# SebastianAment/CompressedSensing.jl

Hardware: AMD Instinct MI355X
Metric: OMP atoms selected/sec at m=4096,n=65536,k=256 (single-signal sweeps, 2 x 3 signals pipelined) (higher is better)
Workload: dtype f64; 1 GPU; configs[1]: single-signal OMP, A 4096x65536 Float32 Gaussian unit-norm, k=256, planted +-1 256-sparse x0 + noise 5e-3, eps=eps(Float32); signals_per_gpu=78, signals_in_flight=6, collective=none (one rank)

## Files before the change

compressedsensing.jl_amd/_lib.py:

```python
import ctypes as C
import os

import numpy as np

HERE = os.path.dirname(os.path.abspath(__file__))
LIB_PATH = os.path.join(HERE, "csrc", "libcsmp.so")

OK, EINVAL, EDIM, ERANGE, EHIP, ESTATE, ENOMEM, ERCCL, EIO = 0, -1, -2, -3, -4, -5, -6, -7, -8
F32, F64 = 0, 1
HOST, DEVICE, HOST_STREAMED = 0, 1, 2
ALGO_MP, ALGO_OMP, ALGO_GOMP, ALGO_FR, ALGO_SP, ALGO_OMPR = 0, 1, 2, 3, 4, 5
STOP_EPS, STOP_STAG, STOP_FULL = 1, 2, 4
OPT_BATCH_CERT, OPT_BATCH_GRAM, OPT_BATCH_WINDOW, OPT_PIPELINE, OPT_SOLVES_IN_FLIGHT, OPT_SCREENED_SWEEP, OPT_BATCH_SCREEN = 1, 2, 3, 4, 9, 10, 11
OPTIONS = {"batch_cert": OPT_BATCH_CERT, "batch_gram": OPT_BATCH_GRAM, "batch_window": OPT_BATCH_WINDOW, "pipeline": OPT_PIPELINE,
           "solves_in_flight": OPT_SOLVES_IN_FLIGHT, "screened_sweep": OPT_SCREENED_SWEEP, "batch_screen": OPT_BATCH_SCREEN}

i64 = C.c_int64
vp = C.c_void_p

SIGNATURES = {
    "csmp_version": (C.c_int, []),
    "csmp_create": (C.c_int, [C.POINTER(vp), C.c_int]),
    "csmp_destroy": (C.c_int, [vp]),
    "csmp_last_error": (C.c_char_p, [vp]),
# ... 70 lines not shown
    "csmp_profile_enable": (C.c_int, [vp, C.c_int]),
    "csmp_profile_read": (C.c_int, [vp, C.POINTER(i64), C.POINTER(C.c_double), C.c_int]),
    "csmp_bench_sweep": (C.c_int, [vp, C.c_int, C.c_int, C.POINTER(C.c_double)]),
    "csmp_bench_ard_forms": (C.c_int, [vp, C.c_int, C.c_int, C.c_double, C.POINTER(C.c_double), C.POINTER(C.c_double)]),
    "csmp_bp_rowgram": (C.c_int, [vp, vp, C.c_int]),
    "csmp_profile_overhead": (C.c_int, [vp, C.c_int, C.POINTER(C.c_double)]),
    "csmp_live_resources": (C.c_int, [C.POINTER(i64)] * 6),
    "csmp_profile_window": (C.c_int, [vp, C.POINTER(i64), C.POINTER(C.c_double), C.POINTER(C.c_double), C.POINTER(C.c_int)]),
    "csmp_sweep_config": (C.c_int, [vp, C.POINTER(C.c_int), C.POINTER(C.c_int), C.POINTER(C.c_int), C.POINTER(C.c_int), C.POINTER(i64), C.POINTER(C.c_int), C.POINTER(C.c_int)]),
    "csmp_sweep_group": (C.c_int, [vp, C.POINTER(C.c_int)]),
    "csmp_sweep_group_wide": (C.c_int, [vp, C.POINTER(C.c_int)]),
    "csmp_tune": (C.c_int, [vp, C.c_int, i64]),
    "csmp_batch_layout": (C.c_int, [vp, C.POINTER(i64), C.POINTER(C.c_int)]),
    "csmp_batch_screen_kernel": (C.c_char_p, [vp]),
}
TUNE = {"sweep_grid": 2, "sweep_unit": 3, "tick_grid": 4, "batch_budget_mib": 5, "diag_split": 6, "swap_refuse": 7, "rebuild_direct": 8, "sweep_dyn": 9, "tick_order": 10, "claim_pools": 11, "pipelines": 12, "pair_lds_kib": 13, "pair_split": 14, "sweep_lds_kib": 15, "sweep_short": 16, "phase_rows": 17, "fail_alloc": 18, "screen_static": 19, "group_max": 20, "group_wide": 21, "rowgram_scalar": 22}

COMM_ID_BYTES = 128
BABEL_KMAX = 1024
ARD_KMAX = 1024
REWEIGHT_CANDES, REWEIGHT_ARD = 0, 1
BP_CONVERGED, BP_FACTORED = 1, 2
BPD_CONVERGED, BPD_FACTORED = 1, 2
BPD_RHO = 100.0


def live_resources():
    v = [i64(0) for _ in range(6)]
    rc = lib().csmp_live_resources(*[C.byref(x) for x in v])
    if rc != OK:
        raise CsmpError(rc, "csmp_live_resources")
# ... 777 lines not shown
```

compressedsensing.jl_amd/csrc/csmp_kernels.hpp:

```cpp
#pragma once
#include <hip/hip_runtime.h>
#include <type_traits>
#include <stdint.h>

namespace csmp {

constexpr int kWave = 64;
constexpr int kSweepThreads = 256;
constexpr int kCPW = 4;
constexpr int kSlabRows = 64;
constexpr int kQrThreads = 256;

enum : int { STOP_EPS = 1, STOP_STAG = 2, STOP_FULL = 4, STOP_REORTH = 8 };
constexpr int STOP_UNCERTAIN = 256;

struct DevState {
    int nsel;
    int j;
    int cand;
    int go;
    int done;
    int steps;
    int go2;
    int pcount;
// ... 1845 lines not shown
    for (int i = 0; i < R; ++i) acc[0][i] = acc[1][i] = 0.0;
    const int Ni = (int)N;
    double bestv[NS];
    int besti[NS];
    double cst[NS];
    int ccst[NS];
#pragma unroll
    for (int s = 0; s < NS; ++s) {
        bestv[s] = -1.0;
        besti[s] = 0x7fffffff;
        cst[s] = 0.0;
        ccst[s] = -1;
    }
    int cslot = 0;
    auto cv = [&](const int i) { return mo ? p.cvec[kGroupMax + i] : p.cvec[i]; };
    auto flush = [&](const int s) {
        double* dst;
        bool on;
        if (s < S4) {
            dst = (lane & 32) ? cv(2 * s + 1) : cv(2 * s);
            on = (live >> (2 * s + (lane >> 5))) & 1u;
        } else {
            dst = cv(R - 1);
            on = (live >> (R - 1)) & 1u;
        }
        if (on && ccst[s] >= 0) dst[ccst[s]] = cst[s];
        ccst[s] = -1;
    };
    int64_t iq = q0, cq = q0;
    int ib = 0, cb = 0;
// ... 137 lines not shown
            for (int s = 0; s < NS; ++s) {
                double v;
                int col;
                bool mine;
                if (s < S4) {
                    v = row_xsum(xs16(xs32(acc[0][2 * s], acc[0][2 * s + 1]), xs32(acc[1][2 * s], acc[1][2 * s + 1])));
                    col = c0 + ((lane >> 4) & 1);
                    mine = ((lane ^ cslot) & 15) == 0;
                } else {
                    v = xs32(acc[0][R - 1], acc[1][R - 1]);
                    v = row_xsum(xs16(v, v));
                    col = c0 + (lane >> 5);
                    mine = ((lane ^ cslot) & 31) == 0;
                }
                const bool have = col < Ni;
                if (mine) {
                    cst[s] = v;
                    ccst[s] = have ? col : -1;
                }
                const double av = fabs(v);
                if (have && av > bestv[s]) {
                    bestv[s] = av;
                    besti[s] = col;
                }
            }
#pragma unroll
            for (int i = 0; i < R; ++i) acc[0][i] = acc[1][i] = 0.0;
            ++cslot;
            if ((cslot & 15) == 0) {
#pragma unroll
                for (int s = 0; s < S4; ++s) flush(s);
                if (cslot == 32) {
                    if constexpr (NS > S4) flush(S4);
                    cslot = 0;
                }
            }
            cb = 0;
            cq += stride;
        }
        --cleft;
    };
    if (T >= 2 * NB) {
        const int64_t groups = T / NB - 1;
        for (int64_t g = 0; g < groups; ++g) {
#pragma unroll
            for (int d = 0; d < NB; ++d) step(buf[d], std::true_type{});
        }
    }
    while (cleft > 0) {
#pragma unroll
        for (int d = 0; d < NB; ++d) {
            if (cleft == 0) break;
            step(buf[d], std::false_type{});
            if (ileft > 0) issue(buf[d]);
        }
    }
#pragma unroll
    for (int s = 0; s < NS; ++s) flush(s);
#pragma unroll
    for (int s = 0; s < S4; ++s) {
        if ((lane & 15) == 0) {
            const int e = (2 * s + (lane >> 5)) * 4 * NW + wave * 4 + ((lane >> 4) & 1);
            redv[e] = redv[e + 2] = bestv[s];
            redi[e] = redi[e + 2] = besti[s];
        }
    }
    if constexpr (NS > S4)
        argmax_put_rows(redv + (R - 1) * 4 * NW, redi + (R - 1) * 4 * NW, wave, lane, bestv[S4], besti[S4]);
    __syncthreads();
    if (tid < R && (live & (1u << tid)))
        argmax_reduce(redv + tid * 4 * NW, redi + tid * 4 * NW, 4 * NW, p.pval[mo + tid], p.pidx[mo + tid], bid);
}
template <typename TA, int U, int R>
// ... 38 lines not shown
    const int64_t ncol = col0 < N ? (N - 1 - col0) / stride + 1 : 0;
    double bestv[R];
    int besti[R];
    const int nunit = (Mv + UR - 1) / UR;
    const int Mst = nunit * UR;
    VT buf[NB][U];
    double acc[R];
#pragma unroll
    for (int i = 0; i < R; ++i) {
        bestv[i] = -1.0;
        besti[i] = 0x7fffffff;
        acc[i] = 0.0;
    }
    CStage<R> cs;
    cs.init();
    int64_t icol = col0, ccol = col0;
    int ib = 0, cb = 0;
    const int64_t T = ncol * nunit;
    int64_t ileft = T, cleft = T;
    auto issue = [&](VT(&b)[U]) {
        load_unit<TA, U>(A, icol, ld, ib * (U * kWave), nvec, lane, b);
        if (++ib == nunit) {
            ib = 0;
            icol += stride;
        }
        --ileft;
    };
#pragma unroll
    for (int d = 0; d < NB; ++d) {
        if (ileft <= 0) {
// ... 40 lines not shown
            } else {
                const double a0 = (double)b[u].x, a1 = (double)b[u].y;
#pragma unroll
                for (int i = 0; i < R; ++i) {
                    const f64x2* rs = reinterpret_cast<const f64x2*>(lds + (size_t)i * KP);
                    const f64x2 r01 = rs[t * kWave + lane];
                    acc[i] = fma(a0, r01.x, acc[i]);
                    acc[i] = fma(a1, r01.y, acc[i]);
                }
            }
        }
        if (++cb == nunit) {
#pragma unroll
            for (int i = 0; i < R; ++i) {
                const double c = wave_xsum(acc[i]);
                cs.put(lane, i, c);
                const double av = fabs(c);
                if (av > bestv[i]) {
                    bestv[i] = av;
                    besti[i] = (int)ccol;
                }
                acc[i] = 0.0;
            }
            cs.col(lane, ccol);
            cs.next(1, p.cvec, live);
            cb = 0;
            ccol += stride;
        }
        --cleft;
    };
    if (T >= 2 * NB) {
        const int64_t groups = T / NB - 1;
        for (int64_t g = 0; g < groups; ++g) {
#pragma unroll
            for (int d = 0; d < NB; ++d) {
                consume(buf[d]);
                issue(buf[d]);
            }
        }
    }
    while (cleft > 0) {
#pragma unroll
        for (int d = 0; d < NB; ++d) {
            if (cleft == 0) break;
            consume(buf[d]);
            if (ileft > 0) issue(buf[d]);
        }
    }
    cs.flush(p.cvec, live);
#pragma unroll
    for (int i = 0; i < R; ++i) argmax_put_rows(redv + i * 4 * NW, redi + i * 4 * NW, wave, lane, bestv[i], besti[i]);
    __syncthreads();
    if (tid < R && (live & (1u << tid)))
        argmax_reduce(redv + tid * 4 * NW, redi + tid * 4 * NW, 4 * NW, p.pval[tid], p.pidx[tid], bid);
}
template <typename TA, int U, int R>
__global__ __launch_bounds__(kSweepThreads) void k_sweep_multi_w4(const MultiSweep<TA> p) {
    extern __shared__ __attribute__((aligned(16))) double lds[];
    sweep_body_multi_w4<TA, U, 32 / U, R>(p, (int)blockIdx.x, lds);
}

template <typename TA>
struct GroupAppend {
    TickQr2 q2[kWideMax];
// ... 469 lines not shown
```

compressedsensing.jl_amd/csrc/host/batch_plan.hpp:

```cpp
#pragma once
#include <cstdint>
#include <vector>

struct TickStages {
    int z, y, x;
    bool az, ay, ax;
    int64_t tz;
};
static TickStages tick_stages(int64_t n, int64_t k, const int size[3]) {
    TickStages t;
    t.z = (int)(n % 3);
    t.y = (int)((n + 2) % 3);
    t.x = (int)((n + 1) % 3);
    t.tz = (n - t.z) / 3;
    t.az = size[t.z] > 0 && t.tz < k;
    t.ay = size[t.y] > 0 && n >= 1 + t.y && (n - 1 - t.y) / 3 < k;
    t.ax = size[t.x] > 0 && n >= 2 + t.x && (n - 2 - t.x) / 3 < k;
    return t;
}

enum class BatchSchedule {
    Signals,
    One,
    Pairs,
// ... 9 lines not shown
    PlanGroup g[2][3];
};

static std::vector<PlanGroup> even_groups(int64_t nsig, int R) {
    std::vector<PlanGroup> groups;
    if (nsig < 1 || R < 1) return groups;
    const int64_t ngroups = (nsig + R - 1) / R, base = nsig / ngroups, extra = nsig % ngroups;
    int64_t at = 0;
    for (int64_t i = 0; i < ngroups; ++i) {
        groups.push_back({at, (int)(base + (i < extra ? 1 : 0))});
        at += groups.back().size;
    }
    return groups;
}

static std::vector<PlanRound> batch_plan(int64_t nsig, BatchSchedule sched, int R, bool one_pipe = false) {
    std::vector<PlanRound> rounds;
    auto round = [&](RoundForm form) -> PlanRound& {
        rounds.emplace_back();
        rounds.back().form = form;
        return rounds.back();
    };
    int64_t at = 0;
    switch (sched) {
        case BatchSchedule::Signals: break;
        case BatchSchedule::One:
            for (; at < nsig; at += 3) {
                PlanRound& r = round(RoundForm::One);
                for (int g = 0; g < 3 && at + g < nsig; ++g) r.g[0][g] = {at + g, 1};
            }
            break;
// ... 1 lines not shown
            for (; nsig - at >= 6; at += 6) {
                PlanRound& r = round(RoundForm::Pair);
                for (int g = 0; g < 3; ++g) {
                    r.g[0][g] = {at + g, 1};
                    r.g[1][g] = {at + 3 + g, 1};
                }
            }
            for (; nsig - at >= 2; at += 2) {
                PlanRound& r = round(RoundForm::Pair);
                r.g[0][0] = {at, 1};
                r.g[1][0] = {at + 1, 1};
            }
            if (at < nsig) round(RoundForm::One).g[0][0] = {at, 1};
            break;
        case BatchSchedule::Grouped: {
            const std::vector<PlanGroup> groups = even_groups(nsig, R);
            for (size_t i = 0; i < groups.size(); ++i) {
                const size_t per = one_pipe ? 3 : 6;
                if (i % per == 0) round(RoundForm::Grouped);
                if (one_pipe) rounds.back().g[0][i % 3] = groups[i];
                else rounds.back().g[i % 2][(i % 6) / 2] = groups[i];
            }
            break;
        }
    }
    return rounds;
}

struct MpRound {
    PlanGroup g[2];
};
// ... 17 lines not shown
```

compressedsensing.jl_amd/csrc/host/ctx.hpp:

```cpp
static std::string g_create_err;
static constexpr int kRsEqCap = 4096;
static constexpr int kRsSettle = 256;

struct Solver {
    std::vector<int> hpos;
    std::vector<unsigned> hstamp;
    unsigned hgen = 0;
    int kcap = 0, outcap = 0;
    int qcap = 0;
    int64_t ldq = 0;
    int G = 0, Mpad = 0;
    double *b = nullptr, *r = nullptr, *cvec = nullptr, *pval = nullptr;
    int* pidx = nullptr;
    double *Q = nullptr, *R = nullptr, *z = nullptr, *W1 = nullptr, *P1 = nullptr, *P2 = nullptr, *P2s = nullptr, *P1s = nullptr;
    double *avec = nullptr, *vvec = nullptr, *coef = nullptr, *scal = nullptr;
    int *sel = nullptr, *cands = nullptr, *ncands = nullptr;
    double *top_lv = nullptr, *cvals = nullptr;
    int *top_li = nullptr, *rs_gt = nullptr, *rs_eq = nullptr, *rs_work = nullptr;
    RsState* rs = nullptr;
    int top_nb = 0;
    DevState* st = nullptr;
    double* bstage = nullptr;
    int64_t *out_idx = nullptr, *out_order = nullptr, *out_nnz = nullptr;
    double* out_val = nullptr;
// ... 188 lines not shown
    bool sweep_dyn = false;
    int tune_sweep_dyn = 0;
    int tune_pair_lds_kib = 0;
    int tune_pair_split = 0;
    int tune_fail_alloc = 0;
    int tune_pipelines = 0;
    int tune_group_max = 0;
    int sweep_group = 0;
    int tune_group_wide = 0;
    bool wide_refused = false;
    int group_wide = 0;
    int claim_pools = 8;
    int tune_rebuild_direct = 0;
    int tune_swap_refuse = 0;
    int tune_rowgram_scalar = 0;
    int tune_diag_split = 0;
    int64_t tune_batch_budget_mib = 0;
    void* comm = nullptr;
    int comm_rank = 0, comm_world = 1;
    int opt_batch_cert = 1;
    int opt_batch_gram = 0;
    int opt_batch_window = 0;
    int64_t scr_solves = 0, scr_fallbacks = 0;
    int scr_grid = 0;
    double scr_cert_abs = 0.0, scr_cert_rel = 0.0, scr_cert_abs2 = 0.0;
    int scr_kwin = 0;
    int scr_image = 1;
    bool scr_lone = false;
    int opt_screened = 0;
    int opt_batch_screen = 3;
// ... 109 lines not shown
```

compressedsensing.jl_amd/csrc/host/forward.hpp:

```cpp
struct FrPass {
    int nq = 1;
    const double* q1 = nullptr;
    double s1 = -1.0;
    const double* q2 = nullptr;
    double s2 = 1.0;
    int64_t qstride = 0;
    const int* unmark = nullptr;
    int update_only = 0;
};

template <typename TA, int U, bool FULL, int NQ>
static hipError_t fr_sweep_launch_t(csmp_ctx* ctx, const FrPass& ps, int grid, size_t lds, double max_eps, int skipmask) {
    Solver& s = ctx->s;
    auto kern = k_fr_sweep<TA, U, FULL, NQ>;
    if (lds > 64 * 1024) {
        hipError_t e = hipFuncSetAttribute((const void*)kern, hipFuncAttributeMaxDynamicSharedMemorySize, (int)lds);
        if (e != hipSuccess) return e;
    }
    hipLaunchKernelGGL(kern, dim3(grid), dim3(kSweepThreads), lds, ctx->stream, (const TA*)ctx->dA, ctx->ld, ctx->Mv, ctx->N,
                       (const double*)s.r, (const double*)s.Q, s.ldq, ps.q1, ps.s1, ps.q2, ps.s2, ps.unmark, ps.update_only, s.rho2,
                       s.dvec, s.pval, s.pidx, (const int*)s.sel, s.st, max_eps, skipmask);
    return hipGetLastError();
}
template <typename TA, int U, bool FULL>
// ... 310 lines not shown
                        if (!group) continue;
                        const int64_t sgn = r.g[p][g].first + m;
                        a.m[a.n++] = io.member(sv, sgn, sigflags + sgn);
                    }
                if (!group) {
                    PlanRound own = r;
                    for (int g = 0; g < 3; ++g) own.g[1 - p][g].size = 0;
                    CHECK(each_member(own, finish));
                } else if (a.n > 0) {
                    CHECK(twin_rc(ctx, cs[p], launch_finish_group(cs[p], a)));
                }
            }
            return CSMP_OK;
        };
        const int members = wide ? ctx->group_wide : ctx->sweep_group;
        for (const PlanRound& r : batch_plan(nsig, sched, members, wide && ctx->tune_group_wide == 2)) {
            CHECK(each_member(r, init));
            CHECK(ctx->dtype == CSMP_F32 ? run_round<float>(r, ctx, tw, isfr, k, eps, p2) : run_round<double>(r, ctx, tw, isfr, k, eps, p2));
            CHECK(finish_round(r));
        }
        return CSMP_OK;
    };
    if (sched == BatchSchedule::Signals) {
        for (int64_t sgn = 0; sgn < nsig && rc == CSMP_OK; ++sgn) rc = solve_one(sgn, true);
    } else {
        rc = batch_pipelines(ctx, twin, nslots, nslots_wide, 1, ensure, run_plan);
    }
    if (rc == CSMP_OK) {
        std::vector<int> hf((size_t)nsig);
        HIPCHECK(hipMemcpyAsync(hf.data(), sigflags, (size_t)nsig * sizeof(int), hipMemcpyDeviceToHost, ctx->stream));
        HIPCHECK(hipStreamSynchronize(ctx->stream));
// ... 128 lines not shown
```

compressedsensing.jl_amd/csrc/host/measure.hpp:

```cpp
extern "C" int csmp_profile_enable(csmp_ctx* ctx, int on) {
    if (!ctx) return CSMP_EINVAL;
    ctx->prof = on != 0;
    ctx->prof_every = on > 1 ? on : 1;
    ctx->prof_count = 0;
    ctx->prof_first = ctx->prof_last = -1;
    if (ctx->prof) {
        HIPCHECK(hipSetDevice(ctx->dev));
        if (!ctx->prof_ref) HIPCHECK(hipEventCreate(&ctx->prof_ref));
        HIPCHECK(hipEventRecord(ctx->prof_ref, ctx->stream));
    }
    return CSMP_OK;
}

extern "C" int csmp_profile_window(csmp_ctx* ctx, int64_t* launches, double* window_ms, double* mean_launch_ms, int* streams) {
    if (!ctx) return CSMP_EINVAL;
    HIPCHECK(hipSetDevice(ctx->dev));
    HIPCHECK(sync_all(ctx));
    csmp_ctx* cc[2] = {ctx, ctx->twins[0]};
    int64_t n = 0, pairs = 0;
    double t0 = 0.0, t1 = 0.0, dur = 0.0;
    int ns = 0;
    for (csmp_ctx* c : cc) {
        if (!c || c->ev_used < 2 || c->prof_first < 0 || !ctx->prof_ref) continue;
        if (c != ctx) HIPCHECK(hipStreamSynchronize(c->stream));
// ... 73 lines not shown
    std::lock_guard<std::mutex> g(csmp_track::mu);
    int64_t db = 0, pb = 0;
    for (const auto& kv : csmp_track::dev) db += (int64_t)kv.second;
    for (const auto& kv : csmp_track::pinned) pb += (int64_t)kv.second;
    if (device_bytes) *device_bytes = db;
    if (device_blocks) *device_blocks = (int64_t)csmp_track::dev.size();
    if (pinned_bytes) *pinned_bytes = pb;
    if (registered_ranges) *registered_ranges = (int64_t)csmp_track::registered.load();
    if (events) *events = (int64_t)csmp_track::events.load();
    if (streams) *streams = (int64_t)csmp_track::streams.load();
    return CSMP_OK;
}

template <typename TA>
static int bench_shared_sweep(csmp_ctx* ctx, int variant, int reps, double* avg_ms) {
    const int R = ctx->sweep_group, wide = variant >= 2;
    if (R < 1) return fail(ctx, CSMP_ESTATE, "bench_sweep: no shared sweep for this dictionary");
    if (wide && ctx->dtype != CSMP_F32) return fail(ctx, CSMP_ESTATE, "bench_sweep: the wide pass serves Float32 dictionaries");
    const int members = wide ? 2 * R : R;
    std::vector<double> r((size_t)ctx->M);
    uint64_t sd = 0x9E3779B97F4A7C15ull;
    int rc = CSMP_OK;
    for (int m = 0; m < members && rc == CSMP_OK; ++m) {
        activate_slot(ctx, 3 * m);
        rc = solver_ensure(ctx, 1, 1, false);
        ctx->s.begun = false;
        for (auto& v : r) {
            sd = sd * 6364136223846793005ull + 1442695040888963407ull;
            v = ((double)(sd >> 11) / 9007199254740992.0) - 0.5;
        }
        if (rc == CSMP_OK) rc = upload_b(ctx, r.data(), CSMP_F64);
    }
    activate_slot(ctx, 0);
    CHECK(rc);
    MultiSweep<TA> p;
    p.A = (const TA*)ctx->dA; p.ld = ctx->ld; p.Mv = ctx->Mv; p.N = ctx->N;
    p.eps = 0.0; p.check_eps = 0; p.skipmask = 0; p.KP = ctx->sweep_KP;
    p.nblk = wide ? wide_nblk(ctx) : pipe_nblk(ctx, ctx->dtype == CSMP_F32 ? kGroupTickGrid : kPairTickGrid);
    multi_members<TA>(ctx, p, 0, members);
    const size_t lds = std::max(sweep_multi_lds_bytes(p.KP, p.n), (size_t)kPairLdsKiB * 1024);
    auto launch = [&]() -> hipError_t { return wide ? wide_launch<TA>(ctx, p, lds, variant == 2) : multi_launch<TA>(ctx, p, lds); };
    for (int i = 0; i < 3; ++i) HIPCHECK(launch());
    struct Events {
        hipEvent_t e[2] = {nullptr, nullptr};
        ~Events() { for (hipEvent_t x : e) if (x) (void)hipEventDestroy(x); }
    } ev;
    HIPCHECK(hipEventCreate(&ev.e[0]));
    HIPCHECK(hipEventCreate(&ev.e[1]));
    HIPCHECK(hipEventRecord(ev.e[0], ctx->stream));
    for (int i = 0; i < reps; ++i) HIPCHECK(launch());
    HIPCHECK(hipEventRecord(ev.e[1], ctx->stream));
    HIPCHECK(hipStreamSynchronize(ctx->stream));
    float ms0 = 0.f;
    HIPCHECK(hipEventElapsedTime(&ms0, ev.e[0], ev.e[1]));
    if (avg_ms) *avg_ms = (double)ms0 / reps;
    return CSMP_OK;
}

extern "C" int csmp_bench_sweep(csmp_ctx* ctx, int variant, int reps, double* avg_ms) {
    if (!ctx || reps < 1) return CSMP_EINVAL;
    if (!ctx->dA) return fail(ctx, CSMP_ESTATE, "no dictionary set (csmp_set_dictionary)");
    if (variant < 0 || variant > 3) return fail(ctx, CSMP_ESTATE, "bench_sweep: variant 0 (the product kernel), 1 (the shared pass), 2 (the wide pass) or 3 (the wide pass, default-policy loads)");
    HIPCHECK(hipSetDevice(ctx->dev));
    if (variant != 0) return ctx->dtype == CSMP_F32 ? bench_shared_sweep<float>(ctx, variant, reps, avg_ms) : bench_shared_sweep<double>(ctx, variant, reps, avg_ms);
    CHECK(solver_ensure(ctx, 1, 1, false));
    ctx->s.begun = false;
    std::vector<double> r((size_t)ctx->M);
    uint64_t sd = 0x9E3779B97F4A7C15ull;
    for (auto& v : r) {
        sd = sd * 6364136223846793005ull + 1442695040888963407ull;
        v = ((double)(sd >> 11) / 9007199254740992.0) - 0.5;
    }
    CHECK(upload_b(ctx, r.data(), CSMP_F64));
    const bool was = ctx->prof;
    ctx->prof = false;
    for (int i = 0; i < 3; ++i) CHECK(launch_sweep(ctx, ctx->s.r, 0.0, 0, 0));
    hipEvent_t e0, e1;
// ... 60 lines not shown
            if (value < 0 || value > 64) return fail(ctx, CSMP_EINVAL, "csmp_tune: sweep_dyn must be 0 (static), 1 (every column claimed) or 2..64 (the last 1 / n of a workgroup's columns claimed)");
            ctx->tune_sweep_dyn = (int)value;
            break;
        case CSMP_TUNE_CLAIM_POOLS:
            if (value < 1 || value > 4096) return fail(ctx, CSMP_EINVAL, "csmp_tune: claim pools must be 1..4096");
            ctx->claim_pools = (int)value;
            return CSMP_OK;
        case CSMP_TUNE_PAIR_LDS_KIB:
            if (value > 159) return fail(ctx, CSMP_EINVAL, "csmp_tune: at most 159 KiB of LDS");
            ctx->tune_pair_lds_kib = (int)value;
            return CSMP_OK;
        case CSMP_TUNE_SCREEN_STATIC: ctx->tune_screen_static = value == 1 ? 1 : 0; return CSMP_OK;
        case CSMP_TUNE_PAIR_SPLIT: ctx->tune_pair_split = value == 1 ? 1 : 0; return CSMP_OK;
        case CSMP_TUNE_FAIL_ALLOC: ctx->tune_fail_alloc = (int)value; return CSMP_OK;
        case CSMP_TUNE_ROWGRAM_SCALAR: ctx->tune_rowgram_scalar = value == 1 ? 1 : 0; return CSMP_OK;
        case CSMP_TUNE_GROUP_MAX:
            if (value > kGroupMax) return fail(ctx, CSMP_EINVAL, "csmp_tune: group_max must be 0 (what the LDS holds) or 1 .. 4");
            ctx->tune_group_max = (int)value;
            break;
        case CSMP_TUNE_GROUP_WIDE:
            if (value > 2) return fail(ctx, CSMP_EINVAL, "csmp_tune: group_wide must be 0 (wide groups where they apply), 1 (off) or 2 (wide groups, three to a round on ONE pipeline)");
            ctx->tune_group_wide = (int)value;
            break;
        case CSMP_TUNE_PIPELINES:
            if (value > 3) return fail(ctx, CSMP_EINVAL, "csmp_tune: pipelines must be 0 (automatic), 1, 2 or 3");
            ctx->tune_pipelines = (int)value;
            return CSMP_OK;
        case CSMP_TUNE_TICK_ORDER: ctx->tick_sweep_first = value != 0; return CSMP_OK;
        case CSMP_TUNE_REBUILD_DIRECT: ctx->tune_rebuild_direct = value ? 1 : 0; return CSMP_OK;
        case CSMP_TUNE_SWAP_REFUSE: ctx->tune_swap_refuse = value ? 1 : 0; return CSMP_OK;
// ... 12 lines not shown
```

compressedsensing.jl_amd/csrc/host/mp_batch.hpp:

```cpp
constexpr bool kMpSplitLone = false;
template <typename TA>
static int mp_group_step(csmp_ctx* ctx, int size, int nblk, int nblk_wide, size_t lds_sweep) {
    CHECK(shared_pass_launch<TA>(ctx, 0, size, 0.0, 0, 0, nblk, nblk_wide, lds_sweep));
    const bool wide = size > kGroupMax;
    MpGroup g;
    g.n = size;
    for (int m = 0; m < kWideMax; ++m) {
        const Solver& s = *slot_ptr(ctx, 3 * std::min(m, size - 1));
        g.r[m] = s.r; g.cvec[m] = s.cvec; g.pval[m] = s.pval; g.pidx[m] = s.pidx; g.st[m] = s.st; g.sel[m] = s.sel; g.z[m] = s.z;
        g.cap[m] = s.kcap;
        g.nblk[m] = wide ? nblk_wide / 2 : nblk;
    }
    const int wgs = ((int)ctx->M + 255) / 256;
    hipLaunchKernelGGL(k_mp_group<TA>, dim3((unsigned)(size * wgs)), dim3(256), 0, ctx->stream, (const TA*)ctx->dA, ctx->ld, (int)ctx->M, ctx->N, g, wgs);
    HIPCHECK(hipGetLastError());
    return CSMP_OK;
}

static int mp_emit(csmp_ctx* ctx, const BatchIO& io, int64_t first, int size) {
    MpEmit e;
    e.n = size;
    for (int m = 0; m < kWideMax; ++m) {
        const int mm = std::min(m, size - 1);
        const Solver& s = *slot_ptr(ctx, 3 * mm);
// ... 72 lines not shown
```

compressedsensing.jl_amd/csrc/host/omp.hpp:

```cpp
template <typename TA>
static TickSweep<TA> tick_sweep_params(csmp_ctx* ctx, Solver& s, double eps, int check_eps, int skipmask, int nblk, int active) {
    TickSweep<TA> p;
    p.claim = p.claim_next = nullptr;
    p.npools = ctx->claim_pools | (ctx->tune_sweep_dyn << 16);
    if (active && ctx->sweep_dyn) claim_sets(s, p.claim, p.claim_next);
    p.A = (const TA*)ctx->dA; p.ld = ctx->ld; p.Mv = ctx->Mv; p.N = ctx->N;
    p.r = s.r; p.cvec = s.cvec; p.pval = s.pval; p.pidx = s.pidx; p.st = s.st;
    p.eps = eps; p.check_eps = check_eps; p.skipmask = skipmask; p.nblk = nblk; p.active = active; p.KP = ctx->sweep_KP;
    p.pcap = ctx->sweep_pcap;
    return p;
}
template <typename TA>
static TickQr1<TA> tick_qr1_params(csmp_ctx* ctx, const Solver& s, int skipmask, int nblk_sweep, int jh, int active) {
    TickQr1<TA> p;
    p.A = (const TA*)ctx->dA; p.ld = ctx->ld; p.M = (int)ctx->M;
    p.Q = s.Q; p.ldq = s.ldq; p.st = s.st; p.avec = s.avec; p.P1 = s.P1;
    p.G = s.G; p.kcap = s.kcap; p.jpad = qr_jpad(jh); p.mode = 1;
    p.pval = s.pval; p.pidx = s.pidx; p.nblk_sweep = nblk_sweep;
    p.cands = s.cands; p.ncands = s.ncands; p.which = 0; p.sel = s.sel; p.skipmask = skipmask;
    p.r = s.r; p.P1s = s.P1s; p.jh = jh; p.active = active;
    return p;
}
static TickQr2 tick_qr2_params(csmp_ctx* ctx, const Solver& s, int jh, int optimistic, int active) {
    TickQr2 p;
// ... 138 lines not shown
        if (p.nblk < 16 || p.nblk % 16 != 0 || p.n1 < 1 || p.n1 > p.n || p.n > kGroupMax) return hipErrorInvalidValue;
        switch (p.n) {
            case 1: return go(k_sweep_wide<TA, 4, 1, NT>);
            case 2: return go(k_sweep_wide<TA, 4, 2, NT>);
            case 3: return go(k_sweep_wide<TA, 4, 3, NT>);
            default: return go(k_sweep_wide<TA, 4, 4, NT>);
        }
    }
}
constexpr bool kWideNt = false;
template <typename TA>
static hipError_t wide_launch(csmp_ctx* ctx, const MultiSweep<TA>& p, size_t lds, bool nt = kWideNt) {
    return nt ? wide_launch_nt<TA, true>(ctx, p, lds) : wide_launch_nt<TA, false>(ctx, p, lds);
}
template <typename TA>
static void multi_members(csmp_ctx* ctx, MultiSweep<TA>& p, int slot0, int size) {
    const bool wide = size > kGroupMax;
    p.n = wide ? (size + 1) / 2 : size;
    p.n1 = wide ? size / 2 : 0;
    for (int e = 0; e < kWideMax; ++e) {
        const int h = e / kGroupMax, i = e % kGroupMax;
        const int m = h == 0 || !wide ? std::min(i, p.n - 1) : p.n + std::min(i, p.n1 - 1);
        const Solver& s = *slot_ptr(ctx, slot0 + 3 * m);
        p.r[e] = s.r; p.cvec[e] = s.cvec; p.pval[e] = s.pval; p.pidx[e] = s.pidx; p.st[e] = s.st;
    }
}
template <typename TA>
static hipError_t multi_launch(csmp_ctx* ctx, const MultiSweep<TA>& p, size_t lds) {
    if constexpr (Vec<TA>::n == 2) {
        switch (ctx->sweep_U) {
            case 16: return multi_launch_u<TA, 16>(ctx, p, lds);
            case 8: return multi_launch_u<TA, 8>(ctx, p, lds);
            default: return multi_launch_u<TA, 4>(ctx, p, lds);
        }
    }
    return multi_launch_u<TA, 4>(ctx, p, lds);
}
template <typename TA>
static int shared_pass_launch(csmp_ctx* ctx, int slot0, int size, double eps, int check_eps, int skipmask, int nblk, int nblk_wide,
                              size_t lds_sweep) {
    MultiSweep<TA> p;
    p.A = (const TA*)ctx->dA; p.ld = ctx->ld; p.Mv = ctx->Mv; p.N = ctx->N;
    const bool wide = size > kGroupMax;
    p.eps = eps; p.check_eps = check_eps; p.skipmask = skipmask; p.nblk = wide ? nblk_wide : nblk; p.KP = ctx->sweep_KP;
    multi_members<TA>(ctx, p, slot0, size);
    const bool timed = prof_pick(ctx);
    if (timed) CHECK(prof_mark(ctx));
    const size_t lds = std::max(sweep_multi_lds_bytes(p.KP, p.n), lds_sweep);
    HIPCHECK(wide ? wide_launch<TA>(ctx, p, lds) : multi_launch<TA>(ctx, p, lds));
    if (timed) CHECK(prof_mark(ctx));
    return CSMP_OK;
}
template <typename TA>
static int group_pipe_launch(Pipe& gp, int64_t n) {
    csmp_ctx* ctx = gp.ctx;
    const int skip = STOP_EPS | STOP_STAG | STOP_FULL | STOP_REORTH;
    const TickStages t = tick_stages(n, gp.k, gp.size);
    if (t.ay || t.ax) {
        GroupAppend<TA> a;
        a.n2 = t.ax ? gp.size[t.x] : 0;
// ... 1 lines not shown
        for (int m = 0; m < a.n2; ++m) {
            const Solver& s = *slot_ptr(ctx, t.x + 3 * m);
            a.q2[m] = tick_qr2_params(ctx, s, s.jh_last, 1, 1);
        }
        for (int m = 0; m < a.n1; ++m) {
            Solver& s = *slot_ptr(ctx, t.y + 3 * m);
            const int jh1 = qr1_advance(s);
            a.q1[m] = tick_qr1_params<TA>(ctx, s, skip, a.n1 > kGroupMax ? gp.nblk_wide / 2 : gp.nblk, jh1, 1);
        }
        const int G = ctx->s.G;
        auto kern = k_append_group<TA>;
        if (gp.lds > 64 * 1024) HIPCHECK(hipFuncSetAttribute((const void*)kern, hipFuncAttributeMaxDynamicSharedMemorySize, (int)gp.lds));
        hipLaunchKernelGGL(kern, dim3((a.n1 + a.n2) * G), dim3(kSweepThreads), gp.lds, ctx->stream, a, G);
        HIPCHECK(hipGetLastError());
    }
    if (t.az) CHECK(shared_pass_launch<TA>(ctx, t.z, gp.size[t.z], gp.eps, t.tz > 0 ? 1 : 0, skip, gp.nblk, gp.nblk_wide, gp.lds_sweep));
    return CSMP_OK;
}

template <int (*launch)(Pipe&, int64_t)>
static int pipe_ticks(Pipe& a, Pipe* b) {
    for (int64_t n = 0; n < 3 * a.k + 2; ++n) {
        CHECK(launch(a, n));
        if (b) CHECK(twin_rc(a.ctx, b->ctx, launch(*b, n)));
    }
    return CSMP_OK;
}

extern "C" int csmp_omp(csmp_ctx* ctx, const void* b, int b_dtype, int64_t k, double eps, int64_t* idx, double* val,
                        int64_t* nnz, int64_t* order) {
    if (!ctx) return CSMP_EINVAL;
// ... 43 lines not shown
```

compressedsensing.jl_amd/csrc/host/steps_sharding.hpp:

```cpp
static int sp_functor_begin(csmp_ctx* ctx, const void* b, int b_dtype, int64_t k, const int64_t* idx0, const double* val0, int64_t nnz0);
static int sp_functor_update(csmp_ctx* ctx);
static int ompr_functor_begin(csmp_ctx* ctx, const void* b, int b_dtype, int64_t k, int64_t nnz0);
static int ompr_functor_update(csmp_ctx* ctx);
static int twostage_functor_state(csmp_ctx* ctx, int64_t* idx, double* val, int64_t* nnz, double* resnorm, int64_t* order, int* stop);

extern "C" int csmp_solver_begin(csmp_ctx* ctx, int algo, const void* b, int b_dtype, int64_t kcap, const int64_t* idx0,
                                 const double* val0, int64_t nnz0) {
    if (!ctx) return CSMP_EINVAL;
    if (!b || kcap < 1) return fail(ctx, CSMP_EINVAL, "solver_begin: bad arguments");
    if (algo != CSMP_ALGO_MP && algo != CSMP_ALGO_OMP && algo != CSMP_ALGO_GOMP && algo != CSMP_ALGO_FR && algo != CSMP_ALGO_SP && algo != CSMP_ALGO_OMPR)
        return fail(ctx, CSMP_EINVAL, "solver_begin: unknown algo");
    if (!ctx->dA) return fail(ctx, CSMP_ESTATE, "no dictionary set (csmp_set_dictionary)");
    HIPCHECK(hipSetDevice(ctx->dev));
    if (algo == CSMP_ALGO_SP || algo == CSMP_ALGO_OMPR) {
        ctx->s.begun = false;
        CHECK(algo == CSMP_ALGO_SP ? sp_functor_begin(ctx, b, b_dtype, kcap, idx0, val0, nnz0) : ompr_functor_begin(ctx, b, b_dtype, kcap, nnz0));
        ctx->s.algo = algo;
        ctx->s.begun = true;
        return CSMP_OK;
    }
    const int kc = algo == CSMP_ALGO_MP ? (int)kcap : (int)std::min<int64_t>(kcap, ctx->M);
    CHECK(solver_ensure(ctx, kc, kc, algo != CSMP_ALGO_MP));
    if (algo == CSMP_ALGO_FR) CHECK(fr_ensure(ctx));
    CHECK(upload_b(ctx, b, b_dtype));
// ... 44 lines not shown
    dst->tune_sweep_U = src->tune_sweep_U;
    dst->tune_sweep_dyn = src->tune_sweep_dyn;
    dst->tick_sweep_first = src->tick_sweep_first;
    dst->claim_pools = src->claim_pools;
    dst->tune_pipelines = src->tune_pipelines;
    dst->tune_pair_lds_kib = src->tune_pair_lds_kib;
    dst->tune_pair_split = src->tune_pair_split;
    dst->tune_sweep_lds_kib = src->tune_sweep_lds_kib;
    dst->sweep_lds_req = src->sweep_lds_req;
    dst->tune_sweep_short = src->tune_sweep_short;
    dst->tune_screen_static = src->tune_screen_static;
    dst->tune_phase_rows = src->tune_phase_rows;
    dst->tick_nblk = src->tick_nblk;
    dst->tune_swap_refuse = src->tune_swap_refuse;
    dst->tune_rebuild_direct = src->tune_rebuild_direct;
}
extern "C" int csmp_clone(csmp_ctx* src, csmp_ctx** out) {
    if (!src || !out) return CSMP_EINVAL;
    *out = nullptr;
    if (!src->dA) return fail(src, CSMP_ESTATE, "clone: no dictionary set (csmp_set_dictionary)");
    csmp_ctx* c = nullptr;
    const int rc = csmp_create(&c, src->dev);
    if (rc != CSMP_OK) {
        src->err = g_create_err;
        return rc;
    }
    c->dA = src->dA;
    c->ownA = false;
    c->share = src->share;
    if (c->share) c->share->refs += 1;
// ... 75 lines not shown
```

include/csmp_internal.h:

```cpp
#ifndef CSMP_INTERNAL_H
#define CSMP_INTERNAL_H
#include "csmp.h"
#ifdef __cplusplus
extern "C" {
#endif

int csmp_profile_enable(csmp_ctx *ctx, int on);
int csmp_profile_read(csmp_ctx *ctx, int64_t *sweep_launches, double *sweep_ms, int reset);
int csmp_profile_window(csmp_ctx *ctx, int64_t *launches, double *window_ms, double *mean_launch_ms, int *streams);
int csmp_profile_overhead(csmp_ctx *ctx, int reps, double *avg_ms);
int csmp_live_resources(int64_t *device_bytes, int64_t *device_blocks, int64_t *pinned_bytes, int64_t *registered_ranges, int64_t *events,
                        int64_t *streams);
int csmp_bench_sweep(csmp_ctx *ctx, int variant, int reps, double *avg_ms);
int csmp_bench_ard_forms(csmp_ctx *ctx, int variant, int reps, double eps, double *avg_ms, double *max_diff);
int csmp_bp_rowgram(csmp_ctx *ctx, double *G_out, int loc);
int csmp_sweep_config(const csmp_ctx *ctx, int *unit_loads, int *phases, int *workgroups, int *tick_workgroups, int64_t *lds_bytes, int *dynamic,
                      int *columns_per_unit);
int csmp_sweep_group(const csmp_ctx *ctx, int *group_max);
int csmp_sweep_group_wide(const csmp_ctx *ctx, int *group_wide);
#define CSMP_TUNE_SWEEP_GRID 2
#define CSMP_TUNE_SWEEP_UNIT 3
#define CSMP_TUNE_TICK_GRID 4
#define CSMP_TUNE_SWEEP_DYN 9
#define CSMP_TUNE_PIPELINES 12
#define CSMP_TUNE_GROUP_MAX 20
#define CSMP_TUNE_GROUP_WIDE 21
#define CSMP_TUNE_ROWGRAM_SCALAR 22
#define CSMP_TUNE_TICK_ORDER 10
#define CSMP_TUNE_CLAIM_POOLS 11
#define CSMP_TUNE_PAIR_LDS_KIB 13
#define CSMP_TUNE_PAIR_SPLIT 14
#define CSMP_TUNE_SWEEP_LDS_KIB 15
#define CSMP_TUNE_SWEEP_SHORT 16
#define CSMP_TUNE_PHASE_ROWS 17
#define CSMP_TUNE_SCREEN_STATIC 19
#define CSMP_TUNE_FAIL_ALLOC 18
#define CSMP_TUNE_REBUILD_DIRECT 8
#define CSMP_TUNE_SWAP_REFUSE 7
#define CSMP_TUNE_DIAG_SPLIT 6
#define CSMP_TUNE_BATCH_BUDGET_MIB 5
int csmp_tune(csmp_ctx *ctx, int key, int64_t value);

// ... 8 lines not shown
```

Measured before the change: 35170 atoms/s.

## Skip correlation-vector stores in shared sweeps and narrow the last signal group

The shared and wide sweep kernels now skip staging and writing the full correlation vector c when cvec is null, and the OMP tick path passes null unless the pass_c tune is set. Only the argmax is kept, which removes n-length global stores per member per sweep. The grouped batch plan can also make the last group narrow when the signal count leaves a small remainder, so the final round does less wasted work. The risk is that any later consumer of cvec in OMP would read stale values.

```diff
diff --git a/compressedsensing.jl_amd/_lib.py b/compressedsensing.jl_amd/_lib.py
--- a/compressedsensing.jl_amd/_lib.py
+++ b/compressedsensing.jl_amd/_lib.py
@@ -108,7 +108,7 @@
     "csmp_batch_layout": (C.c_int, [vp, C.POINTER(i64), C.POINTER(C.c_int)]),
     "csmp_batch_screen_kernel": (C.c_char_p, [vp]),
 }
-TUNE = {"sweep_grid": 2, "sweep_unit": 3, "tick_grid": 4, "batch_budget_mib": 5, "diag_split": 6, "swap_refuse": 7, "rebuild_direct": 8, "sweep_dyn": 9, "tick_order": 10, "claim_pools": 11, "pipelines": 12, "pair_lds_kib": 13, "pair_split": 14, "sweep_lds_kib": 15, "sweep_short": 16, "phase_rows": 17, "fail_alloc": 18, "screen_static": 19, "group_max": 20, "group_wide": 21, "rowgram_scalar": 22}
+TUNE = {"sweep_grid": 2, "sweep_unit": 3, "tick_grid": 4, "batch_budget_mib": 5, "diag_split": 6, "swap_refuse": 7, "rebuild_direct": 8, "sweep_dyn": 9, "tick_order": 10, "claim_pools": 11, "pipelines": 12, "pair_lds_kib": 13, "pair_split": 14, "sweep_lds_kib": 15, "sweep_short": 16, "phase_rows": 17, "fail_alloc": 18, "screen_static": 19, "group_max": 20, "group_wide": 21, "rowgram_scalar": 22, "pass_c": 23, "group_split": 24}
 
 COMM_ID_BYTES = 128
 BABEL_KMAX = 1024
diff --git a/compressedsensing.jl_amd/csrc/csmp_kernels.hpp b/compressedsensing.jl_amd/csrc/csmp_kernels.hpp
--- a/compressedsensing.jl_amd/csrc/csmp_kernels.hpp
+++ b/compressedsensing.jl_amd/csrc/csmp_kernels.hpp
@@ -1883,6 +1883,7 @@
     }
     int cslot = 0;
     auto cv = [&](const int i) { return mo ? p.cvec[kGroupMax + i] : p.cvec[i]; };
+    const bool wc = p.cvec[0] != nullptr;
     auto flush = [&](const int s) {
         double* dst;
         bool on;
@@ -2050,7 +2051,7 @@
                     mine = ((lane ^ cslot) & 31) == 0;
                 }
                 const bool have = col < Ni;
-                if (mine) {
+                if (wc && mine) {
                     cst[s] = v;
                     ccst[s] = have ? col : -1;
                 }
@@ -2062,13 +2063,15 @@
             }
 #pragma unroll
             for (int i = 0; i < R; ++i) acc[0][i] = acc[1][i] = 0.0;
-            ++cslot;
-            if ((cslot & 15) == 0) {
-#pragma unroll
-                for (int s = 0; s < S4; ++s) flush(s);
-                if (cslot == 32) {
-                    if constexpr (NS > S4) flush(S4);
-                    cslot = 0;
+            if (wc) {
+                ++cslot;
+                if ((cslot & 15) == 0) {
+#pragma unroll
+                    for (int s = 0; s < S4; ++s) flush(s);
+                    if (cslot == 32) {
+                        if constexpr (NS > S4) flush(S4);
+                        cslot = 0;
+                    }
                 }
             }
             cb = 0;
@@ -2091,8 +2094,10 @@
             if (ileft > 0) issue(buf[d]);
         }
     }
-#pragma unroll
-    for (int s = 0; s < NS; ++s) flush(s);
+    if (wc) {
+#pragma unroll
+        for (int s = 0; s < NS; ++s) flush(s);
+    }
 #pragma unroll
     for (int s = 0; s < S4; ++s) {
         if ((lane & 15) == 0) {
@@ -2161,6 +2166,7 @@
     }
     CStage<R> cs;
     cs.init();
+    const bool wc = p.cvec[0] != nullptr;
     int64_t icol = col0, ccol = col0;
     int ib = 0, cb = 0;
     const int64_t T = ncol * nunit;
@@ -2231,7 +2237,7 @@
 #pragma unroll
             for (int i = 0; i < R; ++i) {
                 const double c = wave_xsum(acc[i]);
-                cs.put(lane, i, c);
+                if (wc) cs.put(lane, i, c);
                 const double av = fabs(c);
                 if (av > bestv[i]) {
                     bestv[i] = av;
@@ -2239,8 +2245,10 @@
                 }
                 acc[i] = 0.0;
             }
-            cs.col(lane, ccol);
-            cs.next(1, p.cvec, live);
+            if (wc) {
+                cs.col(lane, ccol);
+                cs.next(1, p.cvec, live);
+            }
             cb = 0;
             ccol += stride;
         }
@@ -2264,7 +2272,7 @@
             if (ileft > 0) issue(buf[d]);
         }
     }
-    cs.flush(p.cvec, live);
+    if (wc) cs.flush(p.cvec, live);
 #pragma unroll
     for (int i = 0; i < R; ++i) argmax_put_rows(redv + i * 4 * NW, redi + i * 4 * NW, wave, lane, bestv[i], besti[i]);
     __syncthreads();
diff --git a/compressedsensing.jl_amd/csrc/host/batch_plan.hpp b/compressedsensing.jl_amd/csrc/host/batch_plan.hpp
--- a/compressedsensing.jl_amd/csrc/host/batch_plan.hpp
+++ b/compressedsensing.jl_amd/csrc/host/batch_plan.hpp
@@ -1,4 +1,5 @@
 #pragma once
+#include <cstddef>
 #include <cstdint>
 #include <vector>
 
@@ -47,7 +48,23 @@
     return groups;
 }
 
-static std::vector<PlanRound> batch_plan(int64_t nsig, BatchSchedule sched, int R, bool one_pipe = false) {
+static std::vector<PlanGroup> narrow_last_groups(int64_t nsig, int R, int narrow, int split = 0) {
+    if (nsig < 1 || R < 1) return {};
+    const int64_t p = (nsig + R - 1) / R;
+    if (split == 1 || narrow < 1 || 2 * narrow > R || p < 2 || nsig > (int64_t)R * (p - 1) + narrow) return even_groups(nsig, R);
+    std::vector<PlanGroup> groups;
+    if (split == 2) {
+        groups = even_groups(nsig - narrow, R);
+    } else {
+        const int64_t last = split == 3 ? nsig - (int64_t)R * (p - 1) : narrow;
+        for (int64_t at = 0, left = nsig - last; left > 0; at += R, left -= R) groups.push_back({at, (int)(left < R ? left : R)});
+        if (split == 3) narrow = (int)last;
+    }
+    groups.push_back({nsig - narrow, narrow});
+    return groups;
+}
+
+static std::vector<PlanRound> batch_plan(int64_t nsig, BatchSchedule sched, int R, bool one_pipe = false, int narrow = 0, int split = 0) {
     std::vector<PlanRound> rounds;
     auto round = [&](RoundForm form) -> PlanRound& {
         rounds.emplace_back();
@@ -79,7 +96,7 @@
             if (at < nsig) round(RoundForm::One).g[0][0] = {at, 1};
             break;
         case BatchSchedule::Grouped: {
-            const std::vector<PlanGroup> groups = even_groups(nsig, R);
+            const std::vector<PlanGroup> groups = narrow > 0 ? narrow_last_groups(nsig, R, narrow, split) : even_groups(nsig, R);
             for (size_t i = 0; i < groups.size(); ++i) {
                 const size_t per = one_pipe ? 3 : 6;
                 if (i % per == 0) round(RoundForm::Grouped);
diff --git a/compressedsensing.jl_amd/csrc/host/ctx.hpp b/compressedsensing.jl_amd/csrc/host/ctx.hpp
--- a/compressedsensing.jl_amd/csrc/host/ctx.hpp
+++ b/compressedsensing.jl_amd/csrc/host/ctx.hpp
@@ -226,6 +226,8 @@
     int tune_rebuild_direct = 0;
     int tune_swap_refuse = 0;
     int tune_rowgram_scalar = 0;
+    int tune_pass_c = 0;
+    int tune_group_split = 0;
     int tune_diag_split = 0;
     int64_t tune_batch_budget_mib = 0;
     void* comm = nullptr;
diff --git a/compressedsensing.jl_amd/csrc/host/forward.hpp b/compressedsensing.jl_amd/csrc/host/forward.hpp
--- a/compressedsensing.jl_amd/csrc/host/forward.hpp
+++ b/compressedsensing.jl_amd/csrc/host/forward.hpp
@@ -348,7 +348,7 @@
             return CSMP_OK;
         };
         const int members = wide ? ctx->group_wide : ctx->sweep_group;
-        for (const PlanRound& r : batch_plan(nsig, sched, members, wide && ctx->tune_group_wide == 2)) {
+        for (const PlanRound& r : batch_plan(nsig, sched, members, wide && ctx->tune_group_wide == 2, wide ? ctx->sweep_group : 0, ctx->tune_group_split)) {
             CHECK(each_member(r, init));
             CHECK(ctx->dtype == CSMP_F32 ? run_round<float>(r, ctx, tw, isfr, k, eps, p2) : run_round<double>(r, ctx, tw, isfr, k, eps, p2));
             CHECK(finish_round(r));
diff --git a/compressedsensing.jl_amd/csrc/host/measure.hpp b/compressedsensing.jl_amd/csrc/host/measure.hpp
--- a/compressedsensing.jl_amd/csrc/host/measure.hpp
+++ b/compressedsensing.jl_amd/csrc/host/measure.hpp
@@ -111,6 +111,8 @@
 
 template <typename TA>
 static int bench_shared_sweep(csmp_ctx* ctx, int variant, int reps, double* avg_ms) {
+    const bool need_c = variant <= 3;
+    if (!need_c) variant = variant == 4 ? 1 : 3;
     const int R = ctx->sweep_group, wide = variant >= 2;
     if (R < 1) return fail(ctx, CSMP_ESTATE, "bench_sweep: no shared sweep for this dictionary");
     if (wide && ctx->dtype != CSMP_F32) return fail(ctx, CSMP_ESTATE, "bench_sweep: the wide pass serves Float32 dictionaries");
@@ -134,7 +136,7 @@
     p.A = (const TA*)ctx->dA; p.ld = ctx->ld; p.Mv = ctx->Mv; p.N = ctx->N;
     p.eps = 0.0; p.check_eps = 0; p.skipmask = 0; p.KP = ctx->sweep_KP;
     p.nblk = wide ? wide_nblk(ctx) : pipe_nblk(ctx, ctx->dtype == CSMP_F32 ? kGroupTickGrid : kPairTickGrid);
-    multi_members<TA>(ctx, p, 0, members);
+    multi_members<TA>(ctx, p, 0, members, need_c);
     const size_t lds = std::max(sweep_multi_lds_bytes(p.KP, p.n), (size_t)kPairLdsKiB * 1024);
     auto launch = [&]() -> hipError_t { return wide ? wide_launch<TA>(ctx, p, lds, variant == 2) : multi_launch<TA>(ctx, p, lds); };
     for (int i = 0; i < 3; ++i) HIPCHECK(launch());
@@ -157,7 +159,7 @@
 extern "C" int csmp_bench_sweep(csmp_ctx* ctx, int variant, int reps, double* avg_ms) {
     if (!ctx || reps < 1) return CSMP_EINVAL;
     if (!ctx->dA) return fail(ctx, CSMP_ESTATE, "no dictionary set (csmp_set_dictionary)");
-    if (variant < 0 || variant > 3) return fail(ctx, CSMP_ESTATE, "bench_sweep: variant 0 (the product kernel), 1 (the shared pass), 2 (the wide pass) or 3 (the wide pass, default-policy loads)");
+    if (variant < 0 || variant > 5) return fail(ctx, CSMP_ESTATE, "bench_sweep: variant 0 (the product kernel), 1 (the shared pass), 2 (the wide pass), 3 (the wide pass, default-policy loads), 4 or 5 (1 or 3 without c stores)");
     HIPCHECK(hipSetDevice(ctx->dev));
     if (variant != 0) return ctx->dtype == CSMP_F32 ? bench_shared_sweep<float>(ctx, variant, reps, avg_ms) : bench_shared_sweep<double>(ctx, variant, reps, avg_ms);
     CHECK(solver_ensure(ctx, 1, 1, false));
@@ -248,6 +250,11 @@
         case CSMP_TUNE_PAIR_SPLIT: ctx->tune_pair_split = value == 1 ? 1 : 0; return CSMP_OK;
         case CSMP_TUNE_FAIL_ALLOC: ctx->tune_fail_alloc = (int)value; return CSMP_OK;
         case CSMP_TUNE_ROWGRAM_SCALAR: ctx->tune_rowgram_scalar = value == 1 ? 1 : 0; return CSMP_OK;
+        case CSMP_TUNE_PASS_C: ctx->tune_pass_c = value == 1 ? 1 : 0; return CSMP_OK;
+        case CSMP_TUNE_GROUP_SPLIT:
+            if (value > 3) return fail(ctx, CSMP_EINVAL, "csmp_tune: group_split must be 0 (a narrow last group where it costs no pass), 1 (even), 2 or 3 (measurements)");
+            ctx->tune_group_split = (int)value;
+            return CSMP_OK;
         case CSMP_TUNE_GROUP_MAX:
             if (value > kGroupMax) return fail(ctx, CSMP_EINVAL, "csmp_tune: group_max must be 0 (what the LDS holds) or 1 .. 4");
             ctx->tune_group_max = (int)value;
diff --git a/compressedsensing.jl_amd/csrc/host/mp_batch.hpp b/compressedsensing.jl_amd/csrc/host/mp_batch.hpp
--- a/compressedsensing.jl_amd/csrc/host/mp_batch.hpp
+++ b/compressedsensing.jl_amd/csrc/host/mp_batch.hpp
@@ -1,7 +1,7 @@
 constexpr bool kMpSplitLone = false;
 template <typename TA>
 static int mp_group_step(csmp_ctx* ctx, int size, int nblk, int nblk_wide, size_t lds_sweep) {
-    CHECK(shared_pass_launch<TA>(ctx, 0, size, 0.0, 0, 0, nblk, nblk_wide, lds_sweep));
+    CHECK(shared_pass_launch<TA>(ctx, 0, size, 0.0, 0, 0, nblk, nblk_wide, lds_sweep, true));
     const bool wide = size > kGroupMax;
     MpGroup g;
     g.n = size;
diff --git a/compressedsensing.jl_amd/csrc/host/omp.hpp b/compressedsensing.jl_amd/csrc/host/omp.hpp
--- a/compressedsensing.jl_amd/csrc/host/omp.hpp
+++ b/compressedsensing.jl_amd/csrc/host/omp.hpp
@@ -176,7 +176,7 @@
     return nt ? wide_launch_nt<TA, true>(ctx, p, lds) : wide_launch_nt<TA, false>(ctx, p, lds);
 }
 template <typename TA>
-static void multi_members(csmp_ctx* ctx, MultiSweep<TA>& p, int slot0, int size) {
+static void multi_members(csmp_ctx* ctx, MultiSweep<TA>& p, int slot0, int size, bool need_c) {
     const bool wide = size > kGroupMax;
     p.n = wide ? (size + 1) / 2 : size;
     p.n1 = wide ? size / 2 : 0;
@@ -184,7 +184,7 @@
         const int h = e / kGroupMax, i = e % kGroupMax;
         const int m = h == 0 || !wide ? std::min(i, p.n - 1) : p.n + std::min(i, p.n1 - 1);
         const Solver& s = *slot_ptr(ctx, slot0 + 3 * m);
-        p.r[e] = s.r; p.cvec[e] = s.cvec; p.pval[e] = s.pval; p.pidx[e] = s.pidx; p.st[e] = s.st;
+        p.r[e] = s.r; p.cvec[e] = need_c ? s.cvec : nullptr; p.pval[e] = s.pval; p.pidx[e] = s.pidx; p.st[e] = s.st;
     }
 }
 template <typename TA>
@@ -200,12 +200,12 @@
 }
 template <typename TA>
 static int shared_pass_launch(csmp_ctx* ctx, int slot0, int size, double eps, int check_eps, int skipmask, int nblk, int nblk_wide,
-                              size_t lds_sweep) {
+                              size_t lds_sweep, bool need_c) {
     MultiSweep<TA> p;
     p.A = (const TA*)ctx->dA; p.ld = ctx->ld; p.Mv = ctx->Mv; p.N = ctx->N;
     const bool wide = size > kGroupMax;
     p.eps = eps; p.check_eps = check_eps; p.skipmask = skipmask; p.nblk = wide ? nblk_wide : nblk; p.KP = ctx->sweep_KP;
-    multi_members<TA>(ctx, p, slot0, size);
+    multi_members<TA>(ctx, p, slot0, size, need_c);
     const bool timed = prof_pick(ctx);
     if (timed) CHECK(prof_mark(ctx));
     const size_t lds = std::max(sweep_multi_lds_bytes(p.KP, p.n), lds_sweep);
@@ -237,7 +237,8 @@
         hipLaunchKernelGGL(kern, dim3((a.n1 + a.n2) * G), dim3(kSweepThreads), gp.lds, ctx->stream, a, G);
         HIPCHECK(hipGetLastError());
     }
-    if (t.az) CHECK(shared_pass_launch<TA>(ctx, t.z, gp.size[t.z], gp.eps, t.tz > 0 ? 1 : 0, skip, gp.nblk, gp.nblk_wide, gp.lds_sweep));
+    if (t.az) CHECK(shared_pass_launch<TA>(ctx, t.z, gp.size[t.z], gp.eps, t.tz > 0 ? 1 : 0, skip, gp.nblk, gp.nblk_wide, gp.lds_sweep,
+                                          ctx->tune_pass_c == 1));
     return CSMP_OK;
 }
 
diff --git a/compressedsensing.jl_amd/csrc/host/steps_sharding.hpp b/compressedsensing.jl_amd/csrc/host/steps_sharding.hpp
--- a/compressedsensing.jl_amd/csrc/host/steps_sharding.hpp
+++ b/compressedsensing.jl_amd/csrc/host/steps_sharding.hpp
@@ -82,6 +82,7 @@
     dst->tick_nblk = src->tick_nblk;
     dst->tune_swap_refuse = src->tune_swap_refuse;
     dst->tune_rebuild_direct = src->tune_rebuild_direct;
+    dst->tune_pass_c = src->tune_pass_c;
 }
 extern "C" int csmp_clone(csmp_ctx* src, csmp_ctx** out) {
     if (!src || !out) return CSMP_EINVAL;
diff --git a/include/csmp_internal.h b/include/csmp_internal.h
--- a/include/csmp_internal.h
+++ b/include/csmp_internal.h
@@ -26,6 +26,8 @@
 #define CSMP_TUNE_GROUP_MAX 20
 #define CSMP_TUNE_GROUP_WIDE 21
 #define CSMP_TUNE_ROWGRAM_SCALAR 22
+#define CSMP_TUNE_PASS_C 23
+#define CSMP_TUNE_GROUP_SPLIT 24
 #define CSMP_TUNE_TICK_ORDER 10
 #define CSMP_TUNE_CLAIM_POOLS 11
 #define CSMP_TUNE_PAIR_LDS_KIB 13
```

After: 35620 atoms/s (median of 6 runs). 1.01x the previous value.
